# shipstone-labs/fhe-icp

Measured on AMD Instinct MI355X. Metric: encrypted compares/sec (PBS/sec), 16-dim, 1/2/4/8 GPU; bit-exact vs CPU, higher is better.
Workload: dtype u64; 1 GPU; batch compare 1 query x 1024 encrypted docs per GPU, 16-dim, n_bits=6 (BASELINE configs[1]) + encrypted threshold (min_similarity 0.5) + top-10; docs_per_gpu=1024, total_docs=1024, dim=16, n_bits=6, msg_bits_P=16, pbs_per_compare=7, keyswitch_per_compare=7, parallelism=shard1

## Files before the change

fhe-icp_amd/csrc/br_v4.h:

```cpp
#pragma once
#include "wave_fft.h"

namespace fhei {
namespace v4 {
using u64 = uint64_t;

constexpr int M = 512, N = 1024, S = 8, K = 2;
constexpr int WPC = K + 1;
constexpr int nthreads(int G) { return 64 * G * WPC; }
constexpr int NTA = 8 * 64;
constexpr int NTB = 7 * 8;
constexpr int NTW = NTA + NTB;
constexpr int NMAX = 1023;
constexpr int SCR = 576;

struct Lay {
  int p[9];
};
constexpr Lay LAYS[3] = {{{6, 7, 8, 0, 1, 2, 3, 4, 5}},
                         {{3, 4, 5, 0, 1, 2, 6, 7, 8}},
                         {{0, 1, 2, 4, 5, 8, 3, 6, 7}}};
enum { LA = 0, LB = 1, LC = 2 };

__host__ __device__ constexpr int jof(int li, int lane, int u) {
  int j = 0;
  for (int b = 0; b < 3; ++b) j |= ((u >> b) & 1) << LAYS[li].p[b];
  for (int b = 0; b < 6; ++b) j |= ((lane >> b) & 1) << LAYS[li].p[3 + b];
  return j;
}

#ifndef FHEICP_ABLDS
#define FHEICP_ABLDS 0
#endif
enum { R2F = 0, R2I = 1, R1F = 2, R1I = 3 };
constexpr int RC[4][5] = {{1, 2, 4, 7, 16}, {2, 4, 8, 16, 31}, {2, 4, 8, 16, 30}, {0, 0, 0, 0, 0}};
__host__ __device__ constexpr int rpos(int r, int j) {
  int p = j;
  for (int k = 0; k < 5; ++k) p += RC[r][k] * ((j >> (4 + k)) & 1);
  return p;
}

__host__ __device__ constexpr int bitrev3(int u) { return ((u & 1) << 2) | (u & 2) | ((u >> 2) & 1); }

__host__ __device__ constexpr int lb_low3(int lane) { return jof(1, lane, 0) & 7; }
__device__ __forceinline__ void fill_tables(c64* twl, const c64* __restrict__ tw4, int tid, int nthr) {
  for (int x = tid; x < NTW; x += nthr) twl[x] = tw4[x];
}

__device__ __forceinline__ void lds_barrier() { asm volatile("s_waitcnt lgkmcnt(0)\n\ts_barrier" ::: "memory"); }

__device__ __forceinline__ uint32_t lds_addr(const void* p) { return (uint32_t)(uintptr_t)p; }
__device__ __forceinline__ void ct_signal(uint32_t* f) {
  uint64_t saved;
  asm volatile(
      "s_mov_b64 %0, exec\n\t"
      "s_mov_b64 exec, 1\n\t"
      "ds_add_u32 %1, %2\n\t"
      "s_mov_b64 exec, %0"
      : "=&s"(saved)
      : "v"(lds_addr(f)), "v"(1u)
      : "memory");
}
__device__ __forceinline__ void ct_wait(const uint32_t* f, uint32_t target) {
  uint32_t tv;
  uint32_t ts;
  asm volatile(
      "1:\n\t"
      "ds_read_b32 %0, %2\n\t"
      "s_waitcnt lgkmcnt(0)\n\t"
      "v_readfirstlane_b32 %1, %0\n\t"
      "s_cmp_lt_u32 %1, %3\n\t"
      "s_cbranch_scc0 2f\n\t"
      "s_sleep 1\n\t"
      "s_branch 1b\n"
      "2:"
      : "=&v"(tv), "=&s"(ts)
      : "v"(lds_addr(f)), "s"(target)
      : "memory", "scc");
}

constexpr double RH = 0.70710678118654752440;

__device__ __forceinline__ void dft8(c64 (&v)[S]) {
#pragma unroll
  for (int u = 0; u < 4; ++u) {
    const c64 X = v[u], Y = v[u + 4];
    v[u] = cadd(X, Y);
    const c64 D = csub(X, Y);
    if (u == 0) v[4] = D;
    if (u == 1) v[5] = {D.x - D.y, D.x + D.y};
    if (u == 2) v[6] = {-D.y, D.x};
    if (u == 3) v[7] = {-(D.x + D.y), D.x - D.y};
  }
#pragma unroll
  for (int q = 0; q < 4; ++q) {
    const int u = ((q >> 1) << 2) | (q & 1);
    const c64 X = v[u], Y = v[u + 2];
    v[u] = cadd(X, Y);
    const c64 D = csub(X, Y);
    v[u + 2] = (u & 1) ? c64{-D.y, D.x} : D;
  }
#pragma unroll
  for (int u = 0; u < S; u += 2) {
    const c64 X = v[u], Y = v[u + 1];
    if (u >= 4) {
      v[u] = {__fma_rn(Y.x, RH, X.x), __fma_rn(Y.y, RH, X.y)};
      v[u + 1] = {__fma_rn(Y.x, -RH, X.x), __fma_rn(Y.y, -RH, X.y)};
    } else {
      v[u] = cadd(X, Y);
      v[u + 1] = csub(X, Y);
    }
  }
}
__device__ __forceinline__ void idft8(c64 (&v)[S]) {
#pragma unroll
  for (int u = 0; u < S; u += 2) {
    const c64 X = v[u], Y = v[u + 1];
    v[u] = cadd(X, Y);
    v[u + 1] = csub(X, Y);
  }
#pragma unroll
  for (int q = 0; q < 4; ++q) {
    const int u = ((q >> 1) << 2) | (q & 1);
    const c64 X = v[u], Y0 = v[u + 2];
    const c64 Y = (u & 1) ? c64{Y0.y, -Y0.x} : Y0;
    v[u] = cadd(X, Y);
    v[u + 2] = csub(X, Y);
  }
#pragma unroll
  for (int u = 0; u < 4; ++u) {
    const c64 X = v[u], Y0 = v[u + 4];
    if (u == 1 || u == 3) {
      const c64 Y = (u == 1) ? c64{Y0.x + Y0.y, Y0.y - Y0.x} : c64{Y0.y - Y0.x, -(Y0.x + Y0.y)};
      v[u] = {__fma_rn(Y.x, RH, X.x), __fma_rn(Y.y, RH, X.y)};
      v[u + 4] = {__fma_rn(Y.x, -RH, X.x), __fma_rn(Y.y, -RH, X.y)};
    } else {
      const c64 Y = (u == 2) ? c64{Y0.y, -Y0.x} : Y0;
      v[u] = cadd(X, Y);
      v[u + 4] = csub(X, Y);
    }
  }
}

template <int PS, bool INV, int DBG = 0, int NR = 0>
__device__ __forceinline__ void lane_tw(c64 (&v)[S], const c64* twl, int lane, c64 wf, const c64* treg = nullptr) {
  constexpr int M0 = PS == 0 ? 0 : 1;
#pragma unroll
  for (int h = 0; h < 2; ++h) {
    const int m0 = h ? 4 : M0, m1 = h ? 7 : 3;
    c64 T[4];
#pragma unroll
    for (int m = m0; m <= m1; ++m)
      T[m - m0] = (DBG & 1)            ? wf
                  : (PS == 0 && m < NR) ? treg[m]
                  : PS == 0             ? twl[m * 64 + lane]
                                        : twl[NTA + (m - 1) * 8 + lb_low3(lane)];
#pragma unroll
    for (int u = 0; u < S; ++u) {
      const int m = bitrev3(u);
      if (m < m0 || m > m1) continue;
      v[u] = INV ? cmulc(v[u], T[m - m0]) : cmul(v[u], T[m - m0]);
    }
  }
}

template <bool INV>
__device__ __forceinline__ void fold8(c64 (&v)[S]) {
  constexpr double C[8] = {1.0, 0.98078528040323044913, 0.92387953251128675613, 0.83146961230254523708,
                           0.70710678118654752440, 0.55557023301960222474, 0.38268343236508977173,
                           0.19509032201612826785};
#pragma unroll
  for (int u = 1; u < S; ++u) {
    const c64 c = {C[u], INV ? -C[8 - u] : C[8 - u]};
    v[u] = cmul(v[u], c);
  }
}

template <int R, int LS, int LT, int DBG = 0>
__device__ __forceinline__ void relayout(c64 (&v)[S], c64* scr, int lane) {
  if constexpr ((DBG & 8) != 0) return;
#pragma unroll
  for (int u = 0; u < S; ++u) scr[rpos(R, jof(LS, lane, u))] = v[u];
#pragma unroll
  for (int u = 0; u < S; ++u) v[u] = scr[rpos(R, jof(LT, lane, u))];
}

__device__ __forceinline__ uint32_t dpp_shr8_hi(uint32_t old, uint32_t src) {
  return (uint32_t)__builtin_amdgcn_update_dpp((int)old, (int)src, 0x118, 0xF, 0xC, false);
}
__device__ __forceinline__ uint32_t dpp_shl8_lo(uint32_t old, uint32_t src) {
  return (uint32_t)__builtin_amdgcn_update_dpp((int)old, (int)src, 0x108, 0xF, 0x3, false);
}
template <int KIND>
__device__ __forceinline__ void swap_pair(double& x, double& y) {
  const uint64_t xb = __builtin_bit_cast(uint64_t, x), yb = __builtin_bit_cast(uint64_t, y);
  uint32_t x0 = (uint32_t)xb, x1 = (uint32_t)(xb >> 32), y0 = (uint32_t)yb, y1 = (uint32_t)(yb >> 32);
  if constexpr (KIND == 0) {
    auto a = __builtin_amdgcn_permlane32_swap(x0, y0, false, false);
    auto b = __builtin_amdgcn_permlane32_swap(x1, y1, false, false);
    x0 = a[0], y0 = a[1], x1 = b[0], y1 = b[1];
  } else if constexpr (KIND == 1) {
    auto a = __builtin_amdgcn_permlane16_swap(x0, y0, false, false);
    auto b = __builtin_amdgcn_permlane16_swap(x1, y1, false, false);
    x0 = a[0], y0 = a[1], x1 = b[0], y1 = b[1];
  } else {
    const uint32_t nx0 = dpp_shr8_hi(x0, y0), nx1 = dpp_shr8_hi(x1, y1);
    const uint32_t ny0 = dpp_shl8_lo(y0, x0), ny1 = dpp_shl8_lo(y1, x1);
    x0 = nx0, x1 = nx1, y0 = ny0, y1 = ny1;
  }
  x = __builtin_bit_cast(double, (uint64_t)x0 | ((uint64_t)x1 << 32));
  y = __builtin_bit_cast(double, (uint64_t)y0 | ((uint64_t)y1 << 32));
}
template <int KIND, int STRIDE>
__device__ __forceinline__ void swap_bit(c64 (&v)[S]) {
#pragma unroll
  for (int u = 0; u < S; ++u) {
    if (u & STRIDE) continue;
    swap_pair<KIND>(v[u].x, v[u + STRIDE].x);
    swap_pair<KIND>(v[u].y, v[u + STRIDE].y);
  }
}
__device__ __forceinline__ void swap_lb(c64 (&v)[S]) {
  swap_bit<0, 4>(v);
  swap_bit<1, 2>(v);
  swap_bit<2, 1>(v);
}
template <int DBG = 0, int NR = 0>
__device__ __forceinline__ void forward(c64 (&v)[S], const c64* twl, c64* scr, int lane, c64 wf = {},
                                        const c64* treg = nullptr) {
  fold8<false>(v);
  dft8(v);
  lane_tw<0, false, DBG, NR>(v, twl, lane, wf, treg);
  if constexpr (FHEICP_ABLDS) relayout<R1F, LA, LB, DBG>(v, scr, lane);
  else if constexpr ((DBG & 8) == 0) swap_lb(v);
  dft8(v);
  lane_tw<1, false, DBG>(v, twl, lane, wf);
  relayout<R2F, LB, LC, DBG>(v, scr, lane);
  dft8(v);
}
template <int DBG = 0, int NR = 0>
__device__ __forceinline__ void inverse(c64 (&v)[S], const c64* twl, c64* scr, int lane, c64 wf = {},
                                        const c64* treg = nullptr) {
  idft8(v);
  relayout<R2I, LC, LB, DBG>(v, scr, lane);
  lane_tw<1, true, DBG>(v, twl, lane, wf);
  idft8(v);
  if constexpr (FHEICP_ABLDS) relayout<R1I, LB, LA, DBG>(v, scr, lane);
  else if constexpr ((DBG & 8) == 0) swap_lb(v);
  lane_tw<0, true, DBG, NR>(v, twl, lane, wf, treg);
  idft8(v);
  fold8<true>(v);
}

template <int DBG = 0, int NR = 0>
__device__ __forceinline__ void inverse_post(c64 (&v)[S], const c64* twl, c64* scr, int lane, c64 wf = {},
                                             const c64* treg = nullptr) {
  lane_tw<1, true, DBG>(v, twl, lane, wf);
  idft8(v);
  if constexpr (FHEICP_ABLDS) relayout<R1I, LB, LA, DBG>(v, scr, lane);
  else if constexpr ((DBG & 8) == 0) swap_lb(v);
  lane_tw<0, true, DBG, NR>(v, twl, lane, wf, treg);
  idft8(v);
  fold8<true>(v);
}

template <bool A32>
struct Acc;
template <>
struct Acc<true> {
  using T = uint32_t;
  static __device__ __forceinline__ T from64(u64 x) { return (T)((x + (1ull << 31)) >> 32); }
  static __device__ __forceinline__ u64 to64(T x) { return (u64)x << 32; }
  static __device__ __forceinline__ T from_f64(double z) {
#ifdef FHEICP_A32_ROUND35
    const double t35 = __fma_rn(z, 4294967296.0, 54043195528445952.0);
    return (T)(uint32_t)__builtin_bit_cast(uint64_t, t35) << 3;
#endif
    const double f = __builtin_amdgcn_fract(z);
#ifdef FHEICP_FMA_ROUND
    const double t = __fma_rn(f, 4294967296.0, 6755399441055744.0);
#else
    const double t = __builtin_ldexp(f, 32) + 6755399441055744.0;
#endif
    return (T)(uint32_t)__builtin_bit_cast(uint64_t, t);
  }
};
template <>
struct Acc<false> {
  using T = u64;
  static __device__ __forceinline__ T from64(u64 x) { return x; }
  static __device__ __forceinline__ u64 to64(T x) { return x; }
  static __device__ __forceinline__ T from_f64(double z, uint32_t add = 0) {
#ifdef FHEICP_TORUS_SPLIT
    return f64_to_torus(__builtin_ldexp(z, 64)) + add;
#endif
    constexpr double M = 6755399441055744.0;
    const double F = __builtin_ldexp(z - __builtin_rint(z), 32);
    const double t1 = F + M;
    const double t2 = __builtin_ldexp(F - (t1 - M), 32) + M;
    const u64 hi = (u64)(uint32_t)__builtin_bit_cast(u64, t1) << 32;
    return hi + (__builtin_bit_cast(u64, t2) - (0x4338000000000000ull - add));
  }
};

}
}
```

fhe-icp_amd/csrc/fheicp.hip:

```cpp
#include <hip/hip_runtime.h>

#include <algorithm>
#include <cmath>
#include <cstdio>
#include <cstdlib>
#include <cstring>
#include <mutex>
#include <random>
#include <string>
#include <vector>

#include "../../include/fhe_icp.h"
#include "../../include/fhe_icp_dev.h"
#include "common.h"
#include "k_client.h"
#include "k_server.h"
#include "k_query.h"
#include "k_pack.h"
#include "k_extprod.h"
#include "k_extprod_q.h"
#include "k_blind_rotate.h"

struct ProfAcc {
  std::vector<std::pair<hipEvent_t, hipEvent_t>> ev;
// ... 306 lines not shown
  while (j1 < R && sched[j1] == 0) ++j1;
  while (j2 > 0 && sched[j2 - 1] == 2) --j2;
  *j1_out = j1;
  *j2_out = j2;
}
static int sign_digits(const fhe_params& p) {
  int d, j1, j2;
  sign_plan(p, &d, &j1, &j2);
  return d;
}

extern "C" {

size_t fhe_bsk_words(const fhe_params* p) {
  return (size_t)p->n * (p->k + 1) * p->pbs_level * (p->k + 1) * p->N;
}
size_t fhe_ksk_words(const fhe_params* p) { return (size_t)p->k * p->N * p->ks_level * (p->n + 1); }
size_t fhe_big_lwe_words(const fhe_params* p) { return (size_t)p->k * p->N + 1; }
size_t fhe_small_lwe_words(const fhe_params* p) { return (size_t)p->n + 1; }

const char* fhe_last_error(const fhe_ctx* ctx) {
  if (ctx) return ctx->err.c_str();
  std::lock_guard<std::mutex> lk(g_err_mu);
  return g_err.c_str();
}

int fhe_get_params(const fhe_ctx* ctx, fhe_params* out) {
  if (!ctx || !out) return FHE_E_ARG;
  *out = ctx->p;
  return FHE_OK;
}

int fhe_ctx_create(const fhe_params* params, int device, fhe_ctx** out) {
  std::string why;
  if (!out) return fail(nullptr, FHE_E_ARG, "out is null");
  *out = nullptr;
  if (validate(params, why)) return fail(nullptr, FHE_E_ARG, why);
  fhe_ctx* ctx = new fhe_ctx();
  ctx->p = *params;
  ctx->device = device;
  if (const char* e = getenv("FHEICP_BR_VARIANT")) {
    const int v = atoi(e);
    ctx->br_variant = (v == 2 || v == 4) ? v : 4;
  }
#ifdef FHEICP_AB
  if (const char* e = getenv("FHEICP_V4_DBG")) ctx->v4_dbg = atoi(e);
  if (const char* e = getenv("FHEICP_V4_G")) {
    const int g = atoi(e);
    ctx->v4_g = (g == 1 || g == 2 || g == 4) ? g : 4;
  }
  if (const char* e = getenv("FHEICP_V4_FL")) ctx->v4_fl = atoi(e) != 0;
  if (const char* e = getenv("FHEICP_V4_A64")) ctx->v4_a64 = atoi(e) != 0;
  if (const char* e = getenv("FHEICP_MB_DBG")) ctx->mb_dbg = atoi(e);
  if (const char* e = getenv("FHEICP_V4S")) ctx->v4s = atoi(e);
#endif
  if (const char* e = getenv("FHEICP_KS_VARIANT")) ctx->ks_variant = atoi(e) == 1 ? 1 : 2;
  if ((params->k * params->N) % 64 != 0 || params->ks_level * params->ks_base_log > 31 ||
      params->ks_base_log > 8 ||
      (double)params->k * params->N * params->ks_level * std::ldexp(1.0, params->ks_base_log - 1) * 128 >= 2147483648.0)
    ctx->ks_variant = 1;
  if (device >= 0) {
    int ndev = 0;
    if (hipGetDeviceCount(&ndev) != hipSuccess || device >= ndev) {
      delete ctx;
      return fail(nullptr, FHE_E_DEVICE, "no HIP device " + std::to_string(device));
    }
    if (hipSetDevice(device) != hipSuccess) {
      delete ctx;
      return fail(nullptr, FHE_E_DEVICE, "hipSetDevice failed");
    }
    const int N = params->N, M = N / 2;
    std::vector<c64> tw(M / 2), twist(M);
    for (int x = 0; x < M / 2; ++x) {
      const long double ang = 2.0L * 3.14159265358979323846264338327950288L * (long double)x / (long double)M;
      tw[x] = {(double)cosl(ang), (double)sinl(ang)};
    }
    for (int t = 0; t < M; ++t) {
      const long double ang = 3.14159265358979323846264338327950288L * (long double)t / (long double)N;
      twist[t] = {(double)cosl(ang), (double)sinl(ang)};
    }
    if (N == 1024) {
      const long double PI = 3.14159265358979323846264338327950288L;
      std::vector<c64> t4(v4::NTW);
      for (int m = 0; m < 8; ++m)
        for (int lane = 0; lane < 64; ++lane) {
          const long double ang = PI * (long double)lane * (long double)(1 + 4 * m) / 1024.0L;
          t4[m * 64 + lane] = {(double)cosl(ang), (double)sinl(ang)};
        }
      for (int m = 1; m < 8; ++m)
        for (int L = 0; L < 8; ++L) {
          const long double ang = 2.0L * PI * (long double)(L * m) / 64.0L;
          t4[v4::NTA + (m - 1) * 8 + L] = {(double)cosl(ang), (double)sinl(ang)};
        }
      std::vector<c64> ps(2 * N);
      for (int x = 0; x < 2 * N; ++x) {
        const long double ang = PI * (long double)x / (long double)N;
        const long double h = sinl(ang / 2);
        ps[mb::psi_pos(x)] = {(double)(-2.0L * h * h), (double)sinl(ang)};
      }
      if (hipMalloc(&ctx->tw4, sizeof(c64) * t4.size()) != hipSuccess ||
          hipMemcpy(ctx->tw4, t4.data(), sizeof(c64) * t4.size(), hipMemcpyHostToDevice) != hipSuccess ||
          hipMalloc(&ctx->psi, sizeof(c64) * ps.size()) != hipSuccess ||
          hipMemcpy(ctx->psi, ps.data(), sizeof(c64) * ps.size(), hipMemcpyHostToDevice) != hipSuccess) {
        fhe_ctx_destroy(ctx);
        return fail(nullptr, FHE_E_DEVICE, "twiddle upload failed");
      }
    }
    if (hipMalloc(&ctx->tw, sizeof(c64) * tw.size()) != hipSuccess ||
        hipMalloc(&ctx->twist, sizeof(c64) * twist.size()) != hipSuccess ||
        hipMemcpy(ctx->tw, tw.data(), sizeof(c64) * tw.size(), hipMemcpyHostToDevice) != hipSuccess ||
        hipMemcpy(ctx->twist, twist.data(), sizeof(c64) * twist.size(), hipMemcpyHostToDevice) != hipSuccess) {
      fhe_ctx_destroy(ctx);
      return fail(nullptr, FHE_E_DEVICE, "table upload failed");
    }
  }
  *out = ctx;
  return FHE_OK;
}

static void free_ev(ProfAcc& a) {
  for (auto& e : a.ev) {
    (void)hipEventDestroy(e.first);
    (void)hipEventDestroy(e.second);
  }
  a.ev.clear();
}

void fhe_ctx_destroy(fhe_ctx* ctx) {
  if (!ctx) return;
  if (ctx->device >= 0) {
    (void)hipSetDevice(ctx->device);
    for (void* ptr : {(void*)ctx->s_small, (void*)ctx->s_big, (void*)ctx->bsk, (void*)ctx->ksk,
                      (void*)ctx->ksk_colsum, (void*)ctx->bsk_fft, (void*)ctx->tw, (void*)ctx->twist, ctx->ws,
                      (void*)ctx->bskf[0], (void*)ctx->bskf[1], (void*)ctx->bskf_fft[0], (void*)ctx->bskf_fft[1],
                      (void*)ctx->bskf[2], (void*)ctx->bskf[3], (void*)ctx->bskf_fft[2], (void*)ctx->bskf_fft[3],
                      (void*)ctx->bskf[4], (void*)ctx->bskf_fft[4],
                      (void*)ctx->ksk8, (void*)ctx->ks_ws, (void*)ctx->ks_ws1, (void*)ctx->tw4, (void*)ctx->bsk_fft_v2,
                      (void*)ctx->psi, (void*)ctx->mb_msg, ctx->lq_ws, (void*)ctx->pk, (void*)ctx->pk8,
                      ctx->pack_ws, ctx->xp_ws, ctx->lsq_cst})
      (void)hipFree(ptr);
    for (hipStream_t s : ctx->lane_st)
      if (s) (void)hipStreamDestroy(s);
    for (hipEvent_t e : ctx->lane_ev)
      if (e) (void)hipEventDestroy(e);
    free_ev(ctx->prof_br);
    for (auto& a : ctx->prof_brf) free_ev(a);
    free_ev(ctx->prof_ks);
    free_ev(ctx->prof_enc);
    free_ev(ctx->prof_lq);
    free_ev(ctx->prof_ls);
    free_ev(ctx->prof_pack);
    free_ev(ctx->prof_xp);
    free_ev(ctx->prof_xq);
  }
  delete ctx;
}

int fhe_set_msg_bits(fhe_ctx* ctx, int32_t msg_bits) {
  if (!ctx) return fail(nullptr, FHE_E_ARG, "null ctx");
  fhe_params q = ctx->p;
  q.msg_bits = msg_bits;
  std::string why;
  if (validate(&q, why)) return fail(ctx, FHE_E_ARG, why);
  ctx->p = q;
  return FHE_OK;
}

static int need_device(fhe_ctx* ctx) {
  if (!ctx) return fail(nullptr, FHE_E_ARG, "null ctx");
  if (ctx->device < 0) return fail(ctx, FHE_E_DEVICE, "host-only context");
  if (hipSetDevice(ctx->device) != hipSuccess) return fail(ctx, FHE_E_DEVICE, "hipSetDevice failed");
  return FHE_OK;
}
static int need_eval_keys(fhe_ctx* ctx) {
  int rc = need_device(ctx);
  if (rc) return rc;
// ... 2718 lines not shown
```

fhe-icp_amd/csrc/k_blind_rotate.h:

```cpp
#pragma once

#include <type_traits>

#include "common.h"
#include "br_m512.h"
#include "br_v4.h"

template <int LOGM, int K, class TV>
__device__ __forceinline__ void br_rotate_row(const u64* __restrict__ small, int n, int L, int beta,
                                              const c64* __restrict__ bsk, const c64* __restrict__ tw,
                                              const c64* __restrict__ twist, TV tv, int mode, u64* __restrict__ out,
                                              u64* __restrict__ ct_v, u64* __restrict__ refreshed,
                                              u64* __restrict__ sign, const int64_t c) {
  using F = WaveFFT<LOGM>;
  constexpr int M = F::M, S = F::S, N = 2 * M;
  constexpr int LOG2N2 = LOGM + 2;
  __shared__ u64 acc[(K + 1) * N];
  __shared__ c64 lds[F::LDS_ELEMS];
  const int l = threadIdx.x;
  const u64* sm = small + (size_t)c * (n + 1);
  const int R = (K + 1) * L;

  const uint32_t bt = modswitch_2n(sm[n], LOG2N2);
  for (int t = l; t < N; t += 64) {
// ... 485 lines not shown
          ct_wait(fW, 3 * (phase + 1));
        } else {
          lds_barrier();
        }
      }
      V4_PRIO(3);
      V4_STAMP(4 + 5 * lv);
#pragma unroll
      for (int ci = 0; ci < K; ++ci) {
        if (ci == 1) V4_PRIO(0);
        const int cin = comp + 1 + ci >= WPC ? comp + 1 + ci - WPC : comp + 1 + ci;
        const c64* fs = ctslots + cin * SCR;
        const int gp = Gi + ((cin * L + lv) * WPC + comp) * M;
#pragma unroll
        for (int hh = 0; hh < 2; ++hh) {
          c64 fv[S / 2], kv[S / 2];
#pragma unroll
          for (int u = 0; u < S / 2; ++u) {
            fv[u] = (DBG & 32) ? v[hh * 4 + u] : fs[(hh * 4 + u) * 64 + lane];
            if constexpr (PF) kv[u] = kx[ci][hh * 4 + u];
            else kv[u] = (DBG & 2) ? c64{wf.x + ci, wf.y + u} : krow(gp, hh * 4 + u);
          }
#pragma unroll
          for (int u = 0; u < S / 2; ++u) cmac(mac[hh * 4 + u], fv[u], kv[u]);
        }
      }
      V4_STAMP(5 + 5 * lv);
      if constexpr ((DBG & 4) == 0) {
        if constexpr (FL) {
          ct_signal(fR);
          ++phase;
        } else {
          lds_barrier();
        }
      }
      V4_PRIO(3);
      V4_STAMP(6 + 5 * lv);
    }
    if constexpr (FL && (DBG & 4) == 0) ct_wait(fR, 3 * phase);
    inverse<DBG>(mac, twl, slot, lane, wf);
    V4_STAMP(12);
#pragma unroll
    for (int u = 0; u < S; ++u) {
      acc[u] += AT::from_f64(mac[u].x);
      acc[u + S] += AT::from_f64(mac[u].y);
    }
    V4_PRIO(br_prio_fine<L>() ? 2 : 0);
    V4_STAMP(13);
    if constexpr ((DBG & 128) != 0) stamp_[15] = __builtin_amdgcn_s_memrealtime();
    if constexpr ((DBG & 128) != 0)
      if (blockIdx.x == 0 && w == 0 && i >= 100 && i < 104 && lane < 16) {
        unsigned long long t_ = 0;
#pragma unroll
        for (int k = 0; k < 16; ++k) t_ = lane == k ? stamp_[k] : t_;
        g_v4_stamps[i - 100][lane] = t_;
      }
  }

  if constexpr ((DBG & 128) != 0)
    if (tid == 0 && blockIdx.x < 2048) g_v4_span[blockIdx.x][1] = __builtin_amdgcn_s_memrealtime();
#pragma unroll
  for (int s = 0; s < 2 * S; ++s) sa[s * 64 + lane] = acc[s];
  asm volatile("s_waitcnt lgkmcnt(0)" ::: "memory");
  if (c < count) {
    const int W = K * N + 1;
    if (comp < K) {
#pragma unroll
      for (int s = 0; s < 2 * S; ++s) {
        const int t = s * 64 + lane;
        const u64 x = t == 0 ? AT::to64(sa[0]) : (u64)0 - AT::to64(sa[N - t]);
        br_emit(mode, x, false, tv, (size_t)c * W + comp * N + t, out, ct_v, refreshed, sign);
      }
    } else if (lane == 0) {
      br_emit(mode, AT::to64(acc[0]), true, tv, (size_t)c * W + K * N, out, ct_v, refreshed, sign);
    }
  }
}

namespace fhei {
#ifndef FHEICP_MB_XPOSE
#define FHEICP_MB_XPOSE 1
#endif
__host__ __device__ constexpr bool mb_xpose(int level) { return FHEICP_MB_XPOSE == 2 || (FHEICP_MB_XPOSE == 1 && level == 1); }
namespace mb {
constexpr int NP_MAX = (v4::NMAX + 1) / 2;
__host__ __device__ constexpr int bitrev9(int j) {
  int r = 0;
  for (int b = 0; b < 9; ++b) r |= ((j >> b) & 1) << (8 - b);
  return r;
}
__host__ __device__ constexpr int exponent(int lane, int u) {
  return (4 * bitrev9(v4::jof(v4::LC, lane, u)) + 1) & 2047;
}
__host__ __device__ constexpr int psi_pos(int x) { return x ^ ((x >> 4) & 15); }
}
}

template <int L, int DBG, int BETA, int AW, class TV = BrTv>
__device__ __forceinline__ void mb_rotate(const u64* __restrict__ small, int64_t count, int n, int beta,
                                          const c64* __restrict__ bsk, const c64* __restrict__ tw4,
                                          const c64* __restrict__ psi, TV tv, int mode, u64* __restrict__ out,
                                          u64* __restrict__ ct_v, u64* __restrict__ refreshed, u64* __restrict__ sign,
                                          const unsigned wg) {
  using namespace v4;
  constexpr bool A32 = AW == 1, A48 = AW == 2;
  using AT = Acc<A32>;
  using T = std::conditional_t<A48, uint32_t, typename AT::T>;
#ifndef FHEICP_MB64_ROLL
#define FHEICP_MB64_ROLL 99
#endif
  constexpr bool ROLL = !A32 && L >= FHEICP_MB64_ROLL;
  constexpr int G = 4, NT = nthreads(G), NPSI = 2 * N;
  constexpr int OFF_TW = NPSI, OFF_X = OFF_TW + NTW, NC64 = OFF_X + G * WPC * SCR;
  __shared__ c64 lds[NC64];
  __shared__ uint32_t atab[mb::NP_MAX][G];
  c64* psil = lds;
  c64* twl = lds + OFF_TW;
  c64* xbuf = lds + OFF_X;
  const int tid = threadIdx.x, lane = tid & 63;
  const int w = __builtin_amdgcn_readfirstlane(tid >> 6);
  const int g = w / WPC, comp = w - g * WPC;
  const int64_t c = (int64_t)wg * G + g;
  c64* slot = xbuf + (g * WPC + comp) * SCR;
  using TS = std::conditional_t<A48, u64, T>;
  TS* sa = reinterpret_cast<TS*>(slot);
  const int np = (n + 1) >> 1;
  const int bta = BETA ? BETA : beta;
  const __amdgpu_buffer_rsrc_t krs = __builtin_amdgcn_make_buffer_rsrc((void*)bsk, (short)0, 0x7fffffff, 0x00020000);
  const int kvoff = (comp * M + 2 * g * 64 + lane) * (int)sizeof(c64);

  fill_tables(twl, tw4, tid, NT);
  for (int x = tid; x < NPSI; x += NT) psil[x] = psi[x];
#ifndef FHEICP_MB_TREG
#define FHEICP_MB_TREG 8
#endif
  constexpr int NR = (L == 1 && A32) ? FHEICP_MB_TREG : 0;
  c64 treg[NR > 0 ? NR : 1];
#pragma unroll
  for (int m = 0; m < NR; ++m) treg[m] = tw4[m * 64 + lane];
  for (int x = tid; x < G * np; x += NT) {
    const int gg = x / np, jj = x - gg * np;
    const int64_t cc = (int64_t)wg * G + gg;
    uint32_t a1 = 0, a2 = 0, e = 1;
    if (cc < count) {
      const u64* sm = small + (size_t)cc * (n + 1);
      a1 = modswitch_2n(sm[2 * jj], 11);
      if (2 * jj + 1 < n) {
        a2 = modswitch_2n(sm[2 * jj + 1], 11);
        e = (modswitch_2n(sm[2 * jj] + sm[2 * jj + 1], 11) - a1 - a2 + 1) & (2 * N - 1);
      }
    }
    atab[jj][gg] = a1 | (e << 11) | (a2 << 16);
  }
  __syncthreads();
  constexpr bool XP = mb_xpose(L);
  const uint32_t eb16 = XP
                            ? ((uint32_t)mb::exponent(16 * g + (lane & 15), 2 * (lane >> 4)) & 2047u) << 4
                            : (((uint32_t)mb::exponent(lane, 0) + 256u * bitrev3(2 * g)) & 2047u) << 4;
  const int fpos = XP ? 2 * (lane >> 4) * 64 + 16 * g + (lane & 15) : 0;

  const int prec = L * bta;
  u64 coff = 0;
  if constexpr (!A32) {
    coff = (u64)1 << (63 - prec);
    for (int l = 0; l < L; ++l) coff += (u64)1 << (64 - prec + l * bta + bta - 1);
  }
  T acc[2 * S];
  uint32_t alo[A48 ? S : 1];
  auto word = [&](int s) -> u64 {
    if constexpr (A48)
      return ((u64)acc[s] << 32) | (s < S ? alo[s] << 16 : alo[s - S] & 0xffff0000u);
    else
      return AT::to64(acc[s]);
  };
  auto set48 = [&](int u, u64 a, u64 b) {
    acc[u] = (uint32_t)(a >> 32);
    acc[u + S] = (uint32_t)(b >> 32);
    alo[u] = __builtin_amdgcn_perm((uint32_t)b, (uint32_t)a, 0x07060302u);
  };
  {
    const uint32_t bt = c < count ? modswitch_2n(small[(size_t)c * (n + 1) + n], 11) : 0;
#pragma unroll
    for (int s = 0; s < 2 * S; ++s) {
      const uint32_t idx = (uint32_t)(s * 64 + lane + bt) & (2 * N - 1);
      if constexpr (A48) {
        if (s < S) {
          const uint32_t idx2 = (uint32_t)((s + S) * 64 + lane + bt) & (2 * N - 1);
          set48(s, (comp == K ? tv_rot(tv, idx, N) : 0) + coff, (comp == K ? tv_rot(tv, idx2, N) : 0) + coff);
        }
      } else if constexpr (A32) {
        acc[s] = comp == K ? AT::from64(tv_rot(tv, idx, N)) : (T)0;
      } else {
        acc[s] = (comp == K ? tv_rot(tv, idx, N) : 0) + coff;
      }
    }
  }

  constexpr int R = WPC * L;
  auto digit_at = [&](int s, int lv) -> double {
    u64 w;
    if constexpr (A48) {
      uint32_t t = s < S ? alo[s] : alo[s - S];
      asm volatile("" : "+v"(t));
      w = ((u64)acc[s] << 32) | (s < S ? t << 16 : t);
    } else {
      w = (u64)acc[s];
    }
    return (double)((int)((uint32_t)(w >> (64 - prec + (L - 1 - lv) * bta)) & ((1u << bta) - 1u)) -
                    (1 << (bta - 1)));
  };
  for (int j = 0; j < np; ++j) {
    [[maybe_unused]] unsigned long long stamp_[16];
    V4_STAMP(0);
    uint32_t aS[G][3];
#pragma unroll
    for (int gg = 0; gg < G; ++gg) {
      const uint32_t aa = __builtin_amdgcn_readfirstlane(atab[j][gg]);
      aS[gg][0] = aa & 0x7ffu;
      aS[gg][1] = aa >> 16;
      aS[gg][2] = (aS[gg][0] + aS[gg][1] + ((aa >> 11) & 3u) - 1u) & (2 * N - 1);
    }
    c64 v[S];
    uint32_t dg[(L > 1 && A32) ? L - 1 : 1][S];
#pragma unroll
    for (int s = 0; s < S; ++s) {
      if constexpr (A32) {
        int d[2][L];
#pragma unroll
        for (int h = 0; h < 2; ++h) decompose_v4<L, true>(acc[s + h * S], bta, d[h]);
        v[s] = {(double)d[0][0], (double)d[1][0]};
#pragma unroll
        for (int l = 1; l < L; ++l) dg[l - 1][s] = (uint32_t)(d[0][l] & 0xffff) | ((uint32_t)d[1][l] << 16);
      } else {
        v[s] = {digit_at(s, 0), digit_at(s + S, 0)};
      }
    }
    V4_STAMP(1);
    if constexpr (br_prio_fine<L>()) MB_PRIO(1);
    c64 o[G][2];
#pragma unroll
    for (int gg = 0; gg < G; ++gg) o[gg][0] = o[gg][1] = {0.0, 0.0};
    const int kjoff = j * 3 * R * WPC * M * (int)sizeof(c64);
    constexpr int UNROLL_LV = ROLL ? 1 : L;
#pragma unroll UNROLL_LV
    for (int lv = 0; lv < L; ++lv) {
      if (lv > 0) {
#pragma unroll
        for (int u = 0; u < S; ++u) {
          if constexpr (A32)
            v[u] = {(double)(int16_t)(dg[lv - 1][u] & 0xffff), (double)((int32_t)dg[lv - 1][u] >> 16)};
          else
            v[u] = {digit_at(u, lv), digit_at(u + S, lv)};
        }
      }
      c64 kb[2][3][WPC];
      auto load = [&](int t, c64 (&k)[3][WPC]) {
#pragma unroll
        for (int Ss = 0; Ss < 3; ++Ss)
#pragma unroll
          for (int r = 0; r < WPC; ++r)
            k[Ss][r] = (DBG & 2) ? c64{0.25 + r, 0.5 * t + Ss}
                                 : __builtin_bit_cast(c64, __builtin_amdgcn_raw_buffer_load_b128(
                                       krs, kvoff, kjoff + (((Ss * R + r * L + lv) * WPC) * M + t * 64) * (int)sizeof(c64), 0));
      };
      forward<0, NR>(v, twl, slot, lane, {}, treg);
      V4_STAMP(2 + 4 * lv);
      if constexpr ((DBG & 64) == 0) {
#pragma unroll
        for (int u = 0; u < S; ++u) slot[u * 64 + lane] = v[u];
      }
      load(0, kb[0]);
      V4_STAMP(3 + 4 * lv);
      lds_barrier();
      MB_PRIO(3);
      V4_STAMP(4 + 4 * lv);
      uint32_t pa[G][3];
#pragma unroll
      for (int t = 0; t < 2; ++t) {
        if (t == 1) {
          MB_PRIO(0);
          load(1, kb[1]);
        }
        const int u = 2 * g + t;
#pragma unroll
        for (int gg = 0; gg < G; ++gg) {
          c64 F[WPC];
#pragma unroll
          for (int r = 0; r < WPC; ++r)
            F[r] = (DBG & 32) ? c64{v[(gg + r) & 7].x, v[(gg + 2 * r + t) & 7].y}
                              : xbuf[(gg * WPC + r) * SCR + (XP ? fpos + t * 64 : u * 64 + lane)];
#pragma unroll
          for (int Ss = 0; Ss < 3; ++Ss) {
            c64 P = {0.0, 0.0};
#pragma unroll
            for (int r = 0; r < WPC; ++r) cmac(P, F[r], kb[t][Ss][r]);
            if (t == 0) {
              const uint32_t pr = __umul24(aS[gg][Ss], eb16);
              pa[gg][Ss] = (pr & 0x7ff0u) ^ ((pr >> 4) & 0xf0u);
            } else {
              pa[gg][Ss] ^= (aS[gg][Ss] & 1u) << 14;
            }
            if constexpr ((DBG & 16) != 0)
              cmac(o[gg][t], c64{__builtin_bit_cast(double, (u64)pa[gg][Ss] | 0x3fe0000000000000ull), 0.25}, P);
            else
              cmac(o[gg][t], *reinterpret_cast<const c64*>(reinterpret_cast<const char*>(psil) + pa[gg][Ss]), P);
          }
        }
      }
      V4_STAMP(5 + 4 * lv);
      lds_barrier();
      MB_PRIO(3);
    }
    c64 ov[S];
    if constexpr (XP) {
#pragma unroll
      for (int gg = 0; gg < G; ++gg)
#pragma unroll
        for (int t = 0; t < 2; ++t) ov[2 * gg + t] = o[gg][t];
      swap_bit<0, 4>(ov);
      swap_bit<1, 2>(ov);
      idft8(ov);
      c64* own = xbuf + ((lane >> 4) * WPC + comp) * SCR + rpos(R2I, jof(LC, 16 * g + (lane & 15), 0));
#pragma unroll
      for (int u = 0; u < S; ++u) own[rpos(R2I, jof(LC, 0, u))] = ov[u];
      lds_barrier();
      MB_PRIO(3);
      V4_STAMP(10);
#pragma unroll
      for (int u = 0; u < S; ++u) ov[u] = slot[rpos(R2I, jof(LB, lane, u))];
      inverse_post<0, NR>(ov, twl, slot, lane, {}, treg);
    } else {
#pragma unroll
      for (int gg = 0; gg < G; ++gg)
#pragma unroll
        for (int t = 0; t < 2; ++t) xbuf[(gg * WPC + comp) * SCR + (2 * g + t) * 64 + lane] = o[gg][t];
      lds_barrier();
      MB_PRIO(3);
      V4_STAMP(10);
#pragma unroll
      for (int u = 0; u < S; ++u) ov[u] = slot[u * 64 + lane];
      inverse<0, NR>(ov, twl, slot, lane, {}, treg);
    }
#pragma unroll
    for (int u = 0; u < S; ++u) {
      if constexpr (A48) {
        set48(u, word(u) + Acc<false>::from_f64(ov[u].x, 0x8000u), word(u + S) + Acc<false>::from_f64(ov[u].y, 0x8000u));
      } else {
        acc[u] += AT::from_f64(ov[u].x);
// ... 332 lines not shown
```

fhe-icp_amd/csrc/wave_fft.h:

```cpp
#pragma once
#include <hip/hip_runtime.h>
#include <stdint.h>

namespace fhei {

struct alignas(16) c64 {
  double x, y;
};

__device__ __forceinline__ c64 cadd(c64 a, c64 b) { return {a.x + b.x, a.y + b.y}; }
__device__ __forceinline__ c64 csub(c64 a, c64 b) { return {a.x - b.x, a.y - b.y}; }
__device__ __forceinline__ c64 cmul(c64 a, c64 b) {
  return {__fma_rn(a.x, b.x, -a.y * b.y), __fma_rn(a.x, b.y, a.y * b.x)};
}
__device__ __forceinline__ c64 cmulc(c64 a, c64 b) {
  return {__fma_rn(a.x, b.x, a.y * b.y), __fma_rn(a.y, b.x, -a.x * b.y)};
}
__device__ __forceinline__ void cmac(c64& acc, c64 a, c64 b) {
  acc.x = __fma_rn(a.x, b.x, __fma_rn(-a.y, b.y, acc.x));
  acc.y = __fma_rn(a.x, b.y, __fma_rn(a.y, b.x, acc.y));
}

__host__ __device__ constexpr int ilog2c(int x) { return x <= 1 ? 0 : 1 + ilog2c(x >> 1); }

__device__ __forceinline__ int lds_pad(int j) { return j + (j >> 3); }

template <int LOGM>
struct WaveFFT {
  static constexpr int M = 1 << LOGM;
  static constexpr int S = M / 64;
  static constexpr int LOGS = ilog2c(S);
  static_assert(S >= 1 && (S & (S - 1)) == 0, "M must be a power of two >= 64");
  static constexpr int LDS_ELEMS = M + M / 8;
  static constexpr int Q_NAT = LOGM - LOGS;

  __device__ __forceinline__ static int jidx(int l, int u, int q) {
    return (l & ((1 << q) - 1)) | (u << q) | ((l >> q) << (q + LOGS));
  }

  __device__ __forceinline__ static void relayout(c64 (&v)[S], int qa, int qb, c64* lds, int l) {
#pragma unroll
    for (int u = 0; u < S; ++u) lds[lds_pad(jidx(l, u, qa))] = v[u];
    __syncthreads();
#pragma unroll
    for (int u = 0; u < S; ++u) v[u] = lds[lds_pad(jidx(l, u, qb))];
    __syncthreads();
  }

  __device__ __forceinline__ static void dif_pass(c64 (&v)[S], int q, int top, const c64* __restrict__ tw, int l) {
#pragma unroll
    for (int b = LOGS - 1; b >= 0; --b) {
      const int bit = q + b;
      if (bit > top) continue;
      const int h = 1 << bit;
#pragma unroll
      for (int u = 0; u < S; ++u) {
        if (u & (1 << b)) continue;
        const int jm = ((l & ((1 << q) - 1)) | ((u & ((1 << b) - 1)) << q));
        const c64 W = tw[jm * (M / 2 / h)];
        const c64 X = v[u], Y = v[u | (1 << b)];
        v[u] = cadd(X, Y);
        v[u | (1 << b)] = cmul(csub(X, Y), W);
      }
    }
  }

  __device__ __forceinline__ static void dit_pass(c64 (&v)[S], int q, int top, const c64* __restrict__ tw, int l) {
#pragma unroll
    for (int b = 0; b < LOGS; ++b) {
      const int bit = q + b;
      if (bit > top) continue;
      const int h = 1 << bit;
#pragma unroll
      for (int u = 0; u < S; ++u) {
        if (u & (1 << b)) continue;
        const int jm = ((l & ((1 << q) - 1)) | ((u & ((1 << b) - 1)) << q));
        const c64 W = tw[jm * (M / 2 / h)];
        const c64 X = v[u], Y = cmulc(v[u | (1 << b)], W);
        v[u] = cadd(X, Y);
        v[u | (1 << b)] = csub(X, Y);
      }
    }
  }

  static constexpr int NPASS = (LOGM + LOGS - 1) / LOGS;
  __host__ __device__ static constexpr int top_of(int p) { return LOGM - 1 - p * LOGS; }
  __host__ __device__ static constexpr int q_of(int p) { return LOGM - (p + 1) * LOGS > 0 ? LOGM - (p + 1) * LOGS : 0; }

  __device__ __forceinline__ static void forward(c64 (&v)[S], const c64* __restrict__ tw, c64* lds, int l) {
    int qprev = Q_NAT;
#pragma unroll
    for (int p = 0; p < NPASS; ++p) {
      const int q = q_of(p), top = top_of(p);
      if (q != qprev) relayout(v, qprev, q, lds, l);
      dif_pass(v, q, top, tw, l);
      qprev = q;
    }
    if (qprev != 0) relayout(v, qprev, 0, lds, l);
  }

  __device__ __forceinline__ static void inverse(c64 (&v)[S], const c64* __restrict__ tw, c64* lds, int l) {
    int qprev = 0;
#pragma unroll
// ... 22 lines not shown
```

Measured before the change: 29970 compares/s.

## Fuse forward FFT twiddles into ratio-based radix-8 butterflies with register-held ratios

```diff
diff --git a/fhe-icp_amd/csrc/br_v4.h b/fhe-icp_amd/csrc/br_v4.h
--- a/fhe-icp_amd/csrc/br_v4.h
+++ b/fhe-icp_amd/csrc/br_v4.h
@@ -9,8 +9,11 @@
 constexpr int WPC = K + 1;
 constexpr int nthreads(int G) { return 64 * G * WPC; }
 constexpr int NTA = 8 * 64;
-constexpr int NTB = 7 * 8;
-constexpr int NTW = NTA + NTB;
+constexpr int NFB = 4 * 8;
+constexpr int NIB = 4 * 8;
+constexpr int NFC = 3 * 64;
+constexpr int OFF_FB = NTA, OFF_IB = OFF_FB + NFB, OFF_FC = OFF_IB + NIB;
+constexpr int NTW = OFF_FC + NFC;
 constexpr int NMAX = 1023;
 constexpr int SCR = 576;
 
@@ -43,6 +46,22 @@
 __host__ __device__ constexpr int bitrev3(int u) { return ((u & 1) << 2) | (u & 2) | ((u >> 2) & 1); }
 
 __host__ __device__ constexpr int lb_low3(int lane) { return jof(1, lane, 0) & 7; }
+inline void make_tables(c64* t) {
+  const long double PI = 3.14159265358979323846264338327950288L;
+  const auto put = [&](int at, long double ang) { t[at] = {(double)cosl(ang), (double)sinl(ang)}; };
+  const auto ratios = [&](int at, int stride, long double a, int nr, int w8) {
+    const long double e[4] = {4 * a, 2 * a, a, a + w8 * 256};
+    for (int r = 0; r < nr; ++r) put(at + r * stride, PI * e[r] / 1024.0L);
+  };
+  for (int m = 0; m < 8; ++m)
+    for (int lane = 0; lane < 64; ++lane) put(m * 64 + lane, PI * (long double)(lane * (1 + 4 * m)) / 1024.0L);
+  for (int h = 0; h < 8; ++h) ratios(OFF_FB + h, 8, 8 * (1 + 4 * bitrev3(h)), 4, 1);
+  for (int L = 0; L < 8; ++L) ratios(OFF_IB + L, 8, -32 * L, 4, -1);
+  for (int lane = 0; lane < 64; ++lane) {
+    const int j = jof(LC, lane, 0);
+    ratios(OFF_FC + lane, 64, 1 + 4 * bitrev3((j >> 6) & 7) + 32 * bitrev3((j >> 3) & 7), 3, 1);
+  }
+}
 __device__ __forceinline__ void fill_tables(c64* twl, const c64* __restrict__ tw4, int tid, int nthr) {
   for (int x = tid; x < NTW; x += nthr) twl[x] = tw4[x];
 }
@@ -81,7 +100,7 @@
 
 constexpr double RH = 0.70710678118654752440;
 
-__device__ __forceinline__ void dft8(c64 (&v)[S]) {
+__host__ __device__ __forceinline__ void dft8(c64 (&v)[S]) {
 #pragma unroll
   for (int u = 0; u < 4; ++u) {
     const c64 X = v[u], Y = v[u + 4];
@@ -104,15 +123,15 @@
   for (int u = 0; u < S; u += 2) {
     const c64 X = v[u], Y = v[u + 1];
     if (u >= 4) {
-      v[u] = {__fma_rn(Y.x, RH, X.x), __fma_rn(Y.y, RH, X.y)};
-      v[u + 1] = {__fma_rn(Y.x, -RH, X.x), __fma_rn(Y.y, -RH, X.y)};
+      v[u] = {fmad(Y.x, RH, X.x), fmad(Y.y, RH, X.y)};
+      v[u + 1] = {fmad(Y.x, -RH, X.x), fmad(Y.y, -RH, X.y)};
     } else {
       v[u] = cadd(X, Y);
       v[u + 1] = csub(X, Y);
     }
   }
 }
-__device__ __forceinline__ void idft8(c64 (&v)[S]) {
+__host__ __device__ __forceinline__ void idft8(c64 (&v)[S]) {
 #pragma unroll
   for (int u = 0; u < S; u += 2) {
     const c64 X = v[u], Y = v[u + 1];
@@ -132,8 +151,8 @@
     const c64 X = v[u], Y0 = v[u + 4];
     if (u == 1 || u == 3) {
       const c64 Y = (u == 1) ? c64{Y0.x + Y0.y, Y0.y - Y0.x} : c64{Y0.y - Y0.x, -(Y0.x + Y0.y)};
-      v[u] = {__fma_rn(Y.x, RH, X.x), __fma_rn(Y.y, RH, X.y)};
-      v[u + 4] = {__fma_rn(Y.x, -RH, X.x), __fma_rn(Y.y, -RH, X.y)};
+      v[u] = {fmad(Y.x, RH, X.x), fmad(Y.y, RH, X.y)};
+      v[u + 4] = {fmad(Y.x, -RH, X.x), fmad(Y.y, -RH, X.y)};
     } else {
       const c64 Y = (u == 2) ? c64{Y0.y, -Y0.x} : Y0;
       v[u] = cadd(X, Y);
@@ -142,30 +161,103 @@
   }
 }
 
-template <int PS, bool INV, int DBG = 0, int NR = 0>
-__device__ __forceinline__ void lane_tw(c64 (&v)[S], const c64* twl, int lane, c64 wf, const c64* treg = nullptr) {
-  constexpr int M0 = PS == 0 ? 0 : 1;
+struct Ratios {
+  c64 q4, q2, q1, q1w;
+  __host__ __device__ c64 r4() const { return q4; }
+  __host__ __device__ c64 r2() const { return q2; }
+  __host__ __device__ c64 r1() const { return q1; }
+  __host__ __device__ c64 r1w(c64) const { return q1w; }
+};
+template <int STRIDE, bool W8>
+struct RatioTab {
+  const c64* t;
+  __host__ __device__ c64 r4() const { return t[0]; }
+  __host__ __device__ c64 r2() const { return t[STRIDE]; }
+  __host__ __device__ c64 r1() const { return t[2 * STRIDE]; }
+  __host__ __device__ c64 r1w(c64 r1) const {
+    if constexpr (W8) return {RH * (r1.x - r1.y), RH * (r1.x + r1.y)};
+    else return t[3 * STRIDE];
+  }
+};
+template <int ROT>
+__host__ __device__ __forceinline__ void bfly_tw(c64& X, c64& Y, c64 r) {
+  const c64 q = ROT == 0 ? r : ROT == 1 ? c64{-r.y, r.x} : c64{r.y, -r.x};
+  const c64 Sv = {fmad(q.x, Y.x, fmad(-q.y, Y.y, X.x)), fmad(q.x, Y.y, fmad(q.y, Y.x, X.y))};
+  Y = {fmad(2.0, X.x, -Sv.x), fmad(2.0, X.y, -Sv.y)};
+  X = Sv;
+}
+template <class R>
+__host__ __device__ __forceinline__ void dft8_tw(c64 (&v)[S], const R& t) {
+  const c64 r4 = t.r4();
+#pragma unroll
+  for (int u = 0; u < 4; ++u) bfly_tw<0>(v[u], v[u + 4], r4);
+  const c64 r2 = t.r2();
+  bfly_tw<0>(v[0], v[2], r2);
+  bfly_tw<0>(v[1], v[3], r2);
+  bfly_tw<1>(v[4], v[6], r2);
+  bfly_tw<1>(v[5], v[7], r2);
+  const c64 r1 = t.r1();
+  bfly_tw<0>(v[0], v[1], r1);
+  bfly_tw<1>(v[2], v[3], r1);
+  const c64 r1w = t.r1w(r1);
+  bfly_tw<0>(v[4], v[5], r1w);
+  bfly_tw<1>(v[6], v[7], r1w);
+}
+template <class R>
+__host__ __device__ __forceinline__ void idft8_tw(c64 (&v)[S], const R& t) {
+  const c64 r4 = t.r4();
+#pragma unroll
+  for (int u = 0; u < S; u += 2) bfly_tw<0>(v[u], v[u + 1], r4);
+  const c64 r2 = t.r2();
+  bfly_tw<0>(v[0], v[2], r2);
+  bfly_tw<3>(v[1], v[3], r2);
+  bfly_tw<0>(v[4], v[6], r2);
+  bfly_tw<3>(v[5], v[7], r2);
+  const c64 r1 = t.r1();
+  bfly_tw<0>(v[0], v[4], r1);
+  bfly_tw<3>(v[2], v[6], r1);
+  const c64 r1w = t.r1w(r1);
+  bfly_tw<0>(v[1], v[5], r1w);
+  bfly_tw<3>(v[3], v[7], r1w);
+}
+__host__ __device__ __forceinline__ void dft8_tw_a(c64 (&v)[S]) {
+  dft8_tw(v, Ratios{{RH, RH},
+                    {0.92387953251128675613, 0.38268343236508977173},
+                    {0.98078528040323044913, 0.19509032201612826785},
+                    {0.55557023301960222474, 0.83146961230254523708}});
+}
+using TabFB = RatioTab<8, false>;
+using TabIB = RatioTab<8, false>;
+using TabFC = RatioTab<64, true>;
+__host__ __device__ __forceinline__ TabFB ratios_fb(const c64* twl, int lane) { return {twl + OFF_FB + (lane >> 3)}; }
+__host__ __device__ __forceinline__ TabIB ratios_ib(const c64* twl, int lane) { return {twl + OFF_IB + lb_low3(lane)}; }
+__host__ __device__ __forceinline__ TabFC ratios_fc(const c64* twl, int lane) { return {twl + OFF_FC + lane}; }
+template <class T>
+__host__ __device__ __forceinline__ Ratios held(const T& t) {
+  const c64 r1 = t.r1();
+  return {t.r4(), t.r2(), r1, t.r1w(r1)};
+}
+
+template <int DBG = 0, int NR = 0>
+__host__ __device__ __forceinline__ void lane_tw(c64 (&v)[S], const c64* twl, int lane, c64 wf,
+                                                 const c64* treg = nullptr) {
 #pragma unroll
   for (int h = 0; h < 2; ++h) {
-    const int m0 = h ? 4 : M0, m1 = h ? 7 : 3;
+    const int m0 = h ? 4 : 0, m1 = h ? 7 : 3;
     c64 T[4];
 #pragma unroll
-    for (int m = m0; m <= m1; ++m)
-      T[m - m0] = (DBG & 1)            ? wf
-                  : (PS == 0 && m < NR) ? treg[m]
-                  : PS == 0             ? twl[m * 64 + lane]
-                                        : twl[NTA + (m - 1) * 8 + lb_low3(lane)];
+    for (int m = m0; m <= m1; ++m) T[m - m0] = (DBG & 1) ? wf : m < NR ? treg[m] : twl[m * 64 + lane];
 #pragma unroll
     for (int u = 0; u < S; ++u) {
       const int m = bitrev3(u);
       if (m < m0 || m > m1) continue;
-      v[u] = INV ? cmulc(v[u], T[m - m0]) : cmul(v[u], T[m - m0]);
+      v[u] = cmulc(v[u], T[m - m0]);
     }
   }
 }
 
 template <bool INV>
-__device__ __forceinline__ void fold8(c64 (&v)[S]) {
+__host__ __device__ __forceinline__ void fold8(c64 (&v)[S]) {
   constexpr double C[8] = {1.0, 0.98078528040323044913, 0.92387953251128675613, 0.83146961230254523708,
                            0.70710678118654752440, 0.55557023301960222474, 0.38268343236508977173,
                            0.19509032201612826785};
@@ -225,43 +317,38 @@
   swap_bit<1, 2>(v);
   swap_bit<2, 1>(v);
 }
-template <int DBG = 0, int NR = 0>
+template <int DBG = 0, bool FR = false>
 __device__ __forceinline__ void forward(c64 (&v)[S], const c64* twl, c64* scr, int lane, c64 wf = {},
-                                        const c64* treg = nullptr) {
-  fold8<false>(v);
-  dft8(v);
-  lane_tw<0, false, DBG, NR>(v, twl, lane, wf, treg);
+                                        const Ratios* freg = nullptr) {
+  dft8_tw_a(v);
   if constexpr (FHEICP_ABLDS) relayout<R1F, LA, LB, DBG>(v, scr, lane);
   else if constexpr ((DBG & 8) == 0) swap_lb(v);
-  dft8(v);
-  lane_tw<1, false, DBG>(v, twl, lane, wf);
+  if constexpr ((DBG & 1) != 0) dft8_tw(v, Ratios{wf, wf, wf, wf});
+  else if constexpr (FR) dft8_tw(v, freg[0]);
+  else dft8_tw(v, ratios_fb(twl, lane));
   relayout<R2F, LB, LC, DBG>(v, scr, lane);
-  dft8(v);
+  if constexpr ((DBG & 1) != 0) dft8_tw(v, Ratios{wf, wf, wf, wf});
+  else if constexpr (FR) dft8_tw(v, freg[1]);
+  else dft8_tw(v, ratios_fc(twl, lane));
+}
+
+template <int DBG = 0, int NR = 0>
+__device__ __forceinline__ void inverse_post(c64 (&v)[S], const c64* twl, c64* scr, int lane, c64 wf = {},
+                                             const c64* treg = nullptr) {
+  if constexpr ((DBG & 1) != 0) idft8_tw(v, Ratios{wf, wf, wf, wf});
+  else idft8_tw(v, ratios_ib(twl, lane));
+  if constexpr (FHEICP_ABLDS) relayout<R1I, LB, LA, DBG>(v, scr, lane);
+  else if constexpr ((DBG & 8) == 0) swap_lb(v);
+  lane_tw<DBG, NR>(v, twl, lane, wf, treg);
+  idft8(v);
+  fold8<true>(v);
 }
 template <int DBG = 0, int NR = 0>
 __device__ __forceinline__ void inverse(c64 (&v)[S], const c64* twl, c64* scr, int lane, c64 wf = {},
                                         const c64* treg = nullptr) {
   idft8(v);
   relayout<R2I, LC, LB, DBG>(v, scr, lane);
-  lane_tw<1, true, DBG>(v, twl, lane, wf);
-  idft8(v);
-  if constexpr (FHEICP_ABLDS) relayout<R1I, LB, LA, DBG>(v, scr, lane);
-  else if constexpr ((DBG & 8) == 0) swap_lb(v);
-  lane_tw<0, true, DBG, NR>(v, twl, lane, wf, treg);
-  idft8(v);
-  fold8<true>(v);
-}
-
-template <int DBG = 0, int NR = 0>
-__device__ __forceinline__ void inverse_post(c64 (&v)[S], const c64* twl, c64* scr, int lane, c64 wf = {},
-                                             const c64* treg = nullptr) {
-  lane_tw<1, true, DBG>(v, twl, lane, wf);
-  idft8(v);
-  if constexpr (FHEICP_ABLDS) relayout<R1I, LB, LA, DBG>(v, scr, lane);
-  else if constexpr ((DBG & 8) == 0) swap_lb(v);
-  lane_tw<0, true, DBG, NR>(v, twl, lane, wf, treg);
-  idft8(v);
-  fold8<true>(v);
+  inverse_post<DBG, NR>(v, twl, scr, lane, wf, treg);
 }
 
 template <bool A32>
@@ -304,4 +391,17 @@
 };
 
 }
-}
+
+namespace mb {
+constexpr int NP_MAX = (v4::NMAX + 1) / 2;
+__host__ __device__ constexpr int bitrev9(int j) {
+  int r = 0;
+  for (int b = 0; b < 9; ++b) r |= ((j >> b) & 1) << (8 - b);
+  return r;
+}
+__host__ __device__ constexpr int exponent(int lane, int u) {
+  return (4 * bitrev9(v4::jof(v4::LC, lane, u)) + 1) & 2047;
+}
+__host__ __device__ constexpr int psi_pos(int x) { return x ^ ((x >> 4) & 15); }
+}
+}
diff --git a/fhe-icp_amd/csrc/fheicp.hip b/fhe-icp_amd/csrc/fheicp.hip
--- a/fhe-icp_amd/csrc/fheicp.hip
+++ b/fhe-icp_amd/csrc/fheicp.hip
@@ -412,16 +412,7 @@
     if (N == 1024) {
       const long double PI = 3.14159265358979323846264338327950288L;
       std::vector<c64> t4(v4::NTW);
-      for (int m = 0; m < 8; ++m)
-        for (int lane = 0; lane < 64; ++lane) {
-          const long double ang = PI * (long double)lane * (long double)(1 + 4 * m) / 1024.0L;
-          t4[m * 64 + lane] = {(double)cosl(ang), (double)sinl(ang)};
-        }
-      for (int m = 1; m < 8; ++m)
-        for (int L = 0; L < 8; ++L) {
-          const long double ang = 2.0L * PI * (long double)(L * m) / 64.0L;
-          t4[v4::NTA + (m - 1) * 8 + L] = {(double)cosl(ang), (double)sinl(ang)};
-        }
+      v4::make_tables(t4.data());
       std::vector<c64> ps(2 * N);
       for (int x = 0; x < 2 * N; ++x) {
         const long double ang = PI * (long double)x / (long double)N;
diff --git a/fhe-icp_amd/csrc/k_blind_rotate.h b/fhe-icp_amd/csrc/k_blind_rotate.h
--- a/fhe-icp_amd/csrc/k_blind_rotate.h
+++ b/fhe-icp_amd/csrc/k_blind_rotate.h
@@ -591,18 +591,6 @@
 #define FHEICP_MB_XPOSE 1
 #endif
 __host__ __device__ constexpr bool mb_xpose(int level) { return FHEICP_MB_XPOSE == 2 || (FHEICP_MB_XPOSE == 1 && level == 1); }
-namespace mb {
-constexpr int NP_MAX = (v4::NMAX + 1) / 2;
-__host__ __device__ constexpr int bitrev9(int j) {
-  int r = 0;
-  for (int b = 0; b < 9; ++b) r |= ((j >> b) & 1) << (8 - b);
-  return r;
-}
-__host__ __device__ constexpr int exponent(int lane, int u) {
-  return (4 * bitrev9(v4::jof(v4::LC, lane, u)) + 1) & 2047;
-}
-__host__ __device__ constexpr int psi_pos(int x) { return x ^ ((x >> 4) & 15); }
-}
 }
 
 template <int L, int DBG, int BETA, int AW, class TV = BrTv>
@@ -641,12 +629,21 @@
   fill_tables(twl, tw4, tid, NT);
   for (int x = tid; x < NPSI; x += NT) psil[x] = psi[x];
 #ifndef FHEICP_MB_TREG
-#define FHEICP_MB_TREG 8
+#define FHEICP_MB_TREG 0
+#endif
+#ifndef FHEICP_MB_FREG
+#define FHEICP_MB_FREG 1
 #endif
   constexpr int NR = (L == 1 && A32) ? FHEICP_MB_TREG : 0;
+  constexpr bool FR = L == 1 && A32 && FHEICP_MB_FREG;
   c64 treg[NR > 0 ? NR : 1];
 #pragma unroll
   for (int m = 0; m < NR; ++m) treg[m] = tw4[m * 64 + lane];
+  Ratios freg[2];
+  if constexpr (FR) {
+    freg[0] = held(ratios_fb(tw4, lane));
+    freg[1] = held(ratios_fc(tw4, lane));
+  }
   for (int x = tid; x < G * np; x += NT) {
     const int gg = x / np, jj = x - gg * np;
     const int64_t cc = (int64_t)wg * G + gg;
@@ -772,7 +769,7 @@
                                  : __builtin_bit_cast(c64, __builtin_amdgcn_raw_buffer_load_b128(
                                        krs, kvoff, kjoff + (((Ss * R + r * L + lv) * WPC) * M + t * 64) * (int)sizeof(c64), 0));
       };
-      forward<0, NR>(v, twl, slot, lane, {}, treg);
+      forward<0, FR>(v, twl, slot, lane, {}, freg);
       V4_STAMP(2 + 4 * lv);
       if constexpr ((DBG & 64) == 0) {
 #pragma unroll
diff --git a/fhe-icp_amd/csrc/wave_fft.h b/fhe-icp_amd/csrc/wave_fft.h
--- a/fhe-icp_amd/csrc/wave_fft.h
+++ b/fhe-icp_amd/csrc/wave_fft.h
@@ -8,17 +8,24 @@
   double x, y;
 };
 
-__device__ __forceinline__ c64 cadd(c64 a, c64 b) { return {a.x + b.x, a.y + b.y}; }
-__device__ __forceinline__ c64 csub(c64 a, c64 b) { return {a.x - b.x, a.y - b.y}; }
-__device__ __forceinline__ c64 cmul(c64 a, c64 b) {
-  return {__fma_rn(a.x, b.x, -a.y * b.y), __fma_rn(a.x, b.y, a.y * b.x)};
+__host__ __device__ __forceinline__ double fmad(double a, double b, double c) {
+#if defined(__HIP_DEVICE_COMPILE__)
+  return __fma_rn(a, b, c);
+#else
+  return fma(a, b, c);
+#endif
 }
-__device__ __forceinline__ c64 cmulc(c64 a, c64 b) {
-  return {__fma_rn(a.x, b.x, a.y * b.y), __fma_rn(a.y, b.x, -a.x * b.y)};
+__host__ __device__ __forceinline__ c64 cadd(c64 a, c64 b) { return {a.x + b.x, a.y + b.y}; }
+__host__ __device__ __forceinline__ c64 csub(c64 a, c64 b) { return {a.x - b.x, a.y - b.y}; }
+__host__ __device__ __forceinline__ c64 cmul(c64 a, c64 b) {
+  return {fmad(a.x, b.x, -a.y * b.y), fmad(a.x, b.y, a.y * b.x)};
 }
-__device__ __forceinline__ void cmac(c64& acc, c64 a, c64 b) {
-  acc.x = __fma_rn(a.x, b.x, __fma_rn(-a.y, b.y, acc.x));
-  acc.y = __fma_rn(a.x, b.y, __fma_rn(a.y, b.x, acc.y));
+__host__ __device__ __forceinline__ c64 cmulc(c64 a, c64 b) {
+  return {fmad(a.x, b.x, a.y * b.y), fmad(a.y, b.x, -a.x * b.y)};
+}
+__host__ __device__ __forceinline__ void cmac(c64& acc, c64 a, c64 b) {
+  acc.x = fmad(a.x, b.x, fmad(-a.y, b.y, acc.x));
+  acc.y = fmad(a.x, b.y, fmad(a.y, b.x, acc.y));
 }
 
 __host__ __device__ constexpr int ilog2c(int x) { return x <= 1 ? 0 : 1 + ilog2c(x >> 1); }
```

New measurement: 30020 compares/s, median of 6. Within noise of the previous version (+0.2%).
